# cmusphinx/pocketsphinx

Measured on NVIDIA H100. Metric: frames/sec senone-eval+Viterbi, higher is better.
Workload: dtype f32->i16/i32

## Files before the change

### pocketsphinx_b200/csrc/psb_hmm.cu

```cuda
#include "psb_hmmctx.cuh"

#include <stdlib.h>
#include <string.h>

#include <algorithm>

#include <vector>


struct psb_phoneloop_s {
    psb_hmmctx_t *c;
    int n_phones, window, beam, pbeam, pip;
    double penalty_weight;
    Stream stream;
    DevBuf<int32_t> d_ssid, d_tmatid;
    DevBuf<uint16_t> d_senid;
    DevBuf<int32_t> d_flags;
};

namespace {

__device__ __forceinline__ void load_hmm(const psb_hmm_t *p, HmmReg &h, int n)
{
#pragma unroll
    for (int i = 0; i < PSB_HMM_MAX_NSTATE; ++i) {
        h.score[i] = i < n ? p->score[i] : PSB_WORST_SCORE;
        h.hist[i] = i < n ? p->history[i] : -1;
        h.senid[i] = i < n ? p->senid[i] : PSB_BAD_SSID;
    }
    h.out_score = p->out_score;
    h.out_hist = p->out_history;
    h.best = p->bestscore;
}

__device__ __forceinline__ void store_hmm(psb_hmm_t *p, const HmmReg &h, int n, bool mpx)
{
#pragma unroll
    for (int i = 0; i < PSB_HMM_MAX_NSTATE; ++i)
        if (i < n) {
            p->score[i] = h.score[i];
            p->history[i] = h.hist[i];
            if (mpx) p->senid[i] = (uint16_t)h.senid[i];
        }
    p->out_score = h.out_score;
    p->out_history = h.out_hist;
    p->bestscore = h.best;
}

__global__ void __launch_bounds__(256)
hmm_eval_aos_kernel(psb_hmm_t *hmms, int n, HmmCtxDev c, const int16_t *__restrict__ senscr, int *best_out)
{
    __shared__ int red[8];
    const int i = blockIdx.x * blockDim.x + threadIdx.x;
    int best = PSB_WORST_SCORE;
    if (i < n) {
        psb_hmm_t *p = hmms + i;
        HmmReg h;
        load_hmm(p, h, c.n_emit);
        const bool mpx = p->mpx != 0;
        best = hmm_step(h, c, p->tmatid, mpx, senscr);
        store_hmm(p, h, c.n_emit, mpx);
    }
    best = __reduce_max_sync(0xffffffffu, best);
    if ((threadIdx.x & 31) == 0) red[threadIdx.x >> 5] = best;
    __syncthreads();
    if (threadIdx.x < 32) {
        int v = threadIdx.x < (blockDim.x >> 5) ? red[threadIdx.x] : PSB_WORST_SCORE;
        v = __reduce_max_sync(0xffffffffu, v);
        if (threadIdx.x == 0) atomicMax(best_out, v);
    }
}

struct PlParams {
    int n_phones, window, beam, pbeam, pip;
    double penalty_weight;
};

template <typename T>
__device__ __forceinline__ T block_reduce_max_pair(T v, int idx, int *sidx, T *sval, int &out_idx)
{
    const unsigned full = 0xffffffffu;
#pragma unroll
    for (int o = 16; o > 0; o >>= 1) {
        T ov = __shfl_xor_sync(full, v, o);
        int oi = __shfl_xor_sync(full, idx, o);
        if (ov > v || (ov == v && oi < idx)) { v = ov; idx = oi; }
    }
    const int warp = threadIdx.x >> 5, lane = threadIdx.x & 31, nw = blockDim.x >> 5;
// ... 294 lines not shown
{
    if (!p) return;
    cudaSetDevice(p->c->device);
    cudaStreamSynchronize(p->stream);
    delete p;
}

int psb_phoneloop_launch(psb_phoneloop_t *p, const int16_t *d_senscr, const int32_t *d_utt_off, int32_t n_utt,
                         int32_t *d_best, int32_t *d_pen, psb_hmm_t *d_final, psb_hmm_t *d_trace, cudaStream_t st)
{
    const int H = p->n_phones, N = p->c->n_emit;
    size_t smem = ((size_t)(2 * N + 4 + p->window) * H + 64) * sizeof(int);
    PSB_REQUIRE(smem <= 227 * 1024, "phone loop with %d HMMs needs %zu bytes of shared memory (max 227 KB)", H, smem);
    PSB_CUDA(cudaFuncSetAttribute(phoneloop_kernel, cudaFuncAttributeMaxDynamicSharedMemorySize, (int)smem));
    int threads = std::min(1024, roundup(H, 32));
    PlParams P;
    P.n_phones = H; P.window = p->window; P.beam = p->beam; P.pbeam = p->pbeam; P.pip = p->pip;
    P.penalty_weight = p->penalty_weight;
    phoneloop_kernel<<<n_utt, threads, smem, st>>>(d_senscr, d_utt_off, dev_ctx(p->c), P, p->d_senid, p->d_tmatid, p->d_ssid,
                                                   d_best, d_pen, d_final, d_trace, p->d_flags);
    PSB_LAUNCH_CHECK();
    return PSB_OK;
}

int psb_phoneloop_n_phones(const psb_phoneloop_t *p) { return p->n_phones; }

extern "C" int psb_phoneloop_run_device(psb_phoneloop_t *p, const int16_t *d_senscr, const int32_t *utt_off,
                                        int32_t n_utt, int32_t *d_best, int32_t *d_pen, psb_hmm_t *final_hmms,
                                        void *batch)
{
    PSB_REQUIRE(p && d_senscr && utt_off && n_utt >= 0, "psb_phoneloop_run_device: bad argument");
    if (n_utt == 0) return PSB_OK;
    int rc = ctx_check_utts("psb_phoneloop_run_device", utt_off, n_utt, d_senscr);
    if (rc) return rc;
    PSB_CUDA(cudaSetDevice(p->c->device));
    cudaStream_t st = batch ? psb_batch_stream((psb_batch_t *)batch) : p->stream;
    DevBuf<int32_t> d_off;
    DevBuf<psb_hmm_t> d_final;
    if ((rc = d_off.reserve((size_t)n_utt + 1))) return rc;
    if (final_hmms && (rc = d_final.reserve((size_t)n_utt * p->n_phones))) return rc;
    PSB_CUDA(cudaMemcpyAsync(d_off, utt_off, (size_t)(n_utt + 1) * 4, cudaMemcpyHostToDevice, st));
    rc = psb_phoneloop_launch(p, d_senscr, d_off, n_utt, d_best, d_pen, d_final, nullptr, st);
    if (!rc && final_hmms) {
        cudaError_t e = cudaMemcpyAsync(final_hmms, d_final, (size_t)n_utt * p->n_phones * sizeof(psb_hmm_t),
                                        cudaMemcpyDeviceToHost, st);
        if (e != cudaSuccess) { psb_set_error("%s", cudaGetErrorString(e)); rc = PSB_ERR_CUDA; }
    }
    cudaStreamSynchronize(st);
    return rc;
}

extern "C" int psb_phoneloop_run_host(psb_phoneloop_t *p, const int16_t *senscr, const int32_t *utt_off, int32_t n_utt,
                                      int32_t *best, int32_t *pen, psb_hmm_t *hmm_trace)
{
    PSB_REQUIRE(p && senscr && utt_off && n_utt >= 0, "psb_phoneloop_run_host: bad argument");
    if (n_utt == 0) return PSB_OK;
    int rc = ctx_check_utts("psb_phoneloop_run_host", utt_off, n_utt, senscr);
    if (rc) return rc;
    PSB_CUDA(cudaSetDevice(p->c->device));
    const size_t total = utt_off[n_utt], H = p->n_phones;
    DevBuf<int16_t> d_scr;
    DevBuf<int32_t> d_off, d_best, d_pen;
    DevBuf<psb_hmm_t> d_tr;
    if ((rc = d_scr.reserve(std::max<size_t>(1, total * p->c->n_sen))) || (rc = d_off.reserve((size_t)n_utt + 1)) ||
        (best && (rc = d_best.reserve(std::max<size_t>(1, total)))) || (pen && (rc = d_pen.reserve(std::max<size_t>(1, total * H)))) ||
        (hmm_trace && (rc = d_tr.reserve(std::max<size_t>(1, total * H)))))
        return rc;
    cudaError_t e = cudaMemcpy(d_scr, senscr, total * p->c->n_sen * 2, cudaMemcpyHostToDevice);
    if (e == cudaSuccess) e = cudaMemcpy(d_off, utt_off, (size_t)(n_utt + 1) * 4, cudaMemcpyHostToDevice);
    if (e == cudaSuccess) {
        rc = psb_phoneloop_launch(p, d_scr, d_off, n_utt, d_best, d_pen, nullptr, d_tr, p->stream);
        if (!rc) e = cudaStreamSynchronize(p->stream);
        if (!rc && e == cudaSuccess && best) e = cudaMemcpy(best, d_best, total * 4, cudaMemcpyDeviceToHost);
        if (!rc && e == cudaSuccess && pen) e = cudaMemcpy(pen, d_pen, total * H * 4, cudaMemcpyDeviceToHost);
        if (!rc && e == cudaSuccess && hmm_trace)
            e = cudaMemcpy(hmm_trace, d_tr, total * H * sizeof(psb_hmm_t), cudaMemcpyDeviceToHost);
    }
    if (e != cudaSuccess) { psb_set_error("psb_phoneloop_run_host: %s", cudaGetErrorString(e)); rc = PSB_ERR_CUDA; }
    return rc;
}

constexpr int HS_V = 4;
constexpr int HS_TS = 512;
constexpr int SWEEP_FR = 2;

struct psb_hmmset_s {
    psb_hmmctx_t *c;
    int64_t n_max, n, pitch;
    int32_t n_seg_max, n_seg;
    int64_t max_seg_len;
    bool any_mpx;
    Stream own_stream;
    cudaStream_t stream;
    DevBuf<int32_t> d_i32;
    DevBuf<uint16_t> d_u16;
    DevBuf<uint8_t> d_mpx;
    DevBuf<int64_t> d_seg_off;
    DevBuf<int64_t> d_seg_base;
    DevBuf<psb_hmm_t> d_aos;
    DevBuf<int32_t> d_snap_i32;
    Event ev[2];
};

namespace {

struct HmmSetDev {
    int32_t *i32;
    uint16_t *u16;
    uint8_t *mpx;
    const int64_t *seg_off, *seg_base;
    int64_t pitch;
    int n_seg;
};

static HmmSetDev dev_set(const psb_hmmset_t *s)
{
    HmmSetDev d;
    d.i32 = s->d_i32; d.u16 = s->d_u16; d.mpx = s->d_mpx; d.seg_off = s->d_seg_off; d.seg_base = s->d_seg_base;
    d.pitch = s->pitch; d.n_seg = s->n_seg;
    return d;
}

template <bool TO_SOA>
__global__ void __launch_bounds__(256)
hmmset_convert_kernel(psb_hmm_t *aos, HmmSetDev s, int64_t n, int ns)
{
    const int64_t a = (int64_t)blockIdx.x * blockDim.x + threadIdx.x;
    if (a >= n) return;
    int lo = 0, hi = s.n_seg;
    while (hi - lo > 1) {
        const int mid = (lo + hi) >> 1;
        if (s.seg_off[mid] <= a) lo = mid; else hi = mid;
    }
    const int64_t i = s.seg_base[lo] + (a - s.seg_off[lo]);
    psb_hmm_t *p = aos + a;
    const int64_t b32 = (i / HS_TS) * (int64_t)(2 * ns + 4) * HS_TS + (i % HS_TS);
    const int64_t b16 = (i / HS_TS) * (int64_t)(ns + 2) * HS_TS + (i % HS_TS);
    int32_t *score = s.i32 + b32, *hist = score + ns * HS_TS, *tail = score + 2 * ns * HS_TS;
    uint16_t *senid = s.u16 + b16, *ids = senid + ns * HS_TS;
    if (TO_SOA) {
        for (int k = 0; k < ns; ++k) {
            score[k * HS_TS] = p->score[k];
            hist[k * HS_TS] = p->history[k];
            senid[k * HS_TS] = p->senid[k];
        }
        tail[0] = p->out_score; tail[HS_TS] = p->out_history; tail[2 * HS_TS] = p->bestscore; tail[3 * HS_TS] = p->frame;
        ids[0] = p->ssid; ids[HS_TS] = (uint16_t)p->tmatid;
        s.mpx[i] = p->mpx;
    }
    else {
        for (int k = 0; k < PSB_HMM_MAX_NSTATE; ++k) {
            p->score[k] = k < ns ? score[k * HS_TS] : 0;
            p->history[k] = k < ns ? hist[k * HS_TS] : 0;
            p->senid[k] = k < ns ? senid[k * HS_TS] : 0;
        }
        p->out_score = tail[0]; p->out_history = tail[HS_TS]; p->bestscore = tail[2 * HS_TS]; p->frame = tail[3 * HS_TS];
        p->ssid = ids[0]; p->tmatid = (int16_t)ids[HS_TS];
        p->mpx = s.mpx[i]; p->n_emit_state = (uint8_t)ns;
        p->ctx = nullptr;
    }
}

__global__ void fill_i32_kernel(int32_t *p, int64_t n, int32_t v)
{
    const int64_t i = (int64_t)blockIdx.x * blockDim.x + threadIdx.x;
    if (i < n) p[i] = v;
}
// ... 96 lines not shown
            reinterpret_cast<int16_t *>(dst + head + body)[threadIdx.x - 32] = row[((head + body) >> 1) + threadIdx.x - 32];
        srow_al = reinterpret_cast<const int16_t *>(dst);
        __syncthreads();
        if (body) mbar_wait(&row_bar, 0u);
    }
    int best = PSB_WORST_SCORE;
    if (live) {
        bool any_mpx = false;
#pragma unroll
        for (int q = 0; q < HS_V; ++q) {
            HmmReg h;
#pragma unroll
            for (int k = 0; k < PSB_HMM_MAX_NSTATE; ++k) {
                const bool in = k < NL && k < ns;
                h.score[k] = in ? comp(sc[k < NL ? k : 0], q) : PSB_WORST_SCORE;
                h.hist[k] = in ? comp(hi[k < NL ? k : 0], q) : -1;
                const unsigned w = (q < 2) ? sid[k < NL ? k : 0].x : sid[k < NL ? k : 0].y;
                h.senid[k] = in ? (int)((q & 1) ? (w >> 16) : (w & 0xffffu)) : PSB_BAD_SSID;
            }
            h.out_score = comp(osc, q);
            h.out_hist = comp(ohi, q);
            h.best = PSB_WORST_SCORE;
            const unsigned tw = (q < 2) ? tm.x : tm.y;
            const int tmatid = (int16_t)((q & 1) ? (tw >> 16) : (tw & 0xffffu));
            const bool mpx = (q == 0 ? mp.x : q == 1 ? mp.y : q == 2 ? mp.z : mp.w) != 0;
            const int b = hmm_step(h, c, tmatid, mpx, srow_al);
            if (j0 + q < n) best = max(best, b);
#pragma unroll
            for (int k = 0; k < NL; ++k)
                if (k < ns) {
                    setc(sc[k], q, h.score[k]);
                    setc(hi[k], q, h.hist[k]);
                    if (mpx) {
                        unsigned &w = (q < 2) ? sid[k].x : sid[k].y;
                        w = (q & 1) ? ((w & 0xffffu) | ((unsigned)h.senid[k] << 16)) : ((w & 0xffff0000u) | ((unsigned)h.senid[k] & 0xffffu));
                        any_mpx = true;
                    }
                }
            setc(osc, q, h.out_score);
            setc(ohi, q, h.out_hist);
            setc(bst, q, h.best);
        }
#pragma unroll
        for (int k = 0; k < NL; ++k)
            if (k < ns) {
                __stcs(reinterpret_cast<int4 *>(score + k * HS_TS), sc[k]);
                __stcs(reinterpret_cast<int4 *>(hist + k * HS_TS), hi[k]);
                if (any_mpx) __stcs(reinterpret_cast<uint2 *>(senid + k * HS_TS), sid[k]);
            }
        __stcs(reinterpret_cast<int4 *>(tail), osc);
        __stcs(reinterpret_cast<int4 *>(tail + HS_TS), ohi);
        __stcs(reinterpret_cast<int4 *>(tail + 2 * HS_TS), bst);
    }
    best = __reduce_max_sync(0xffffffffu, best);
    if ((threadIdx.x & 31) == 0) red[threadIdx.x >> 5] = best;
    __syncthreads();
    if (threadIdx.x < 32) {
        int v = threadIdx.x < (HS_THREADS >> 5) ? red[threadIdx.x] : PSB_WORST_SCORE;
        v = __reduce_max_sync(0xffffffffu, v);
        if (threadIdx.x == 0) atomicMax(best_out + seg, v);
    }
}

__device__ __forceinline__ unsigned cluster_ctarank() { unsigned r; asm volatile("mov.u32 %0, %%cluster_ctarank;" : "=r"(r)); return r; }
__device__ __forceinline__ unsigned cluster_nctarank() { unsigned r; asm volatile("mov.u32 %0, %%cluster_nctarank;" : "=r"(r)); return r; }
__device__ __forceinline__ unsigned mapa_shared(const void *p, unsigned rank)
{
    unsigned r;
    asm volatile("mapa.shared::cluster.u32 %0, %1, %2;" : "=r"(r) : "r"((unsigned)__cvta_generic_to_shared(p)), "r"(rank));
    return r;
}
__device__ __forceinline__ void st_cluster_u32(unsigned addr, unsigned v) { asm volatile("st.shared::cluster.u32 [%0], %1;" :: "r"(addr), "r"(v) : "memory"); }
__device__ __forceinline__ unsigned ld_cluster_u32(unsigned addr) { unsigned v; asm volatile("ld.shared::cluster.u32 %0, [%1];" : "=r"(v) : "r"(addr) : "memory"); return v; }
__device__ __forceinline__ void st_async_v2(unsigned remote_addr, unsigned a, unsigned b, unsigned remote_bar)
{
    asm volatile("st.async.weak.shared::cluster.mbarrier::complete_tx::bytes.v2.b32 [%0], {%1, %2}, [%3];"
                 :: "r"(remote_addr), "r"(a), "r"(b), "r"(remote_bar) : "memory");
}
__device__ __forceinline__ void cluster_sync_all()
{
    asm volatile("barrier.cluster.arrive.release.aligned;\n\tbarrier.cluster.wait.acquire.aligned;" ::: "memory");
}

template <int NS, int V, int THREADS, bool BEAM>
__global__ void __launch_bounds__(THREADS, BEAM ? 1 : 2)
hmmset_sweep_kernel(HmmSetDev s, HmmCtxDev c, const int16_t *__restrict__ senscr, long long rows_total,
                    const int64_t *__restrict__ row0, const int32_t *__restrict__ n_rows, int n_frames,
                    int32_t *__restrict__ best_out, int n_tmat, int buf_bytes, int frame0, int beam, int maxhmmpf,
                    int32_t *__restrict__ n_active_out)
{
    static_assert(!BEAM || THREADS == 256, "the histogram walk maps one bin to one thread");
    constexpr int FR = BEAM ? 1 : SWEEP_FR;
    constexpr int NBUF = BEAM ? 6 : 2 * FR;
    extern __shared__ __align__(128) unsigned char sw_smem[];
    __shared__ __align__(8) uint64_t full[NBUF];
    __shared__ int red[2 * FR][THREADS / 32];
    __shared__ int redc[BEAM ? 2 : 1][THREADS / 32];
    __shared__ __align__(8) int2 cl_slot[BEAM ? 2 : 1][16];
    __shared__ __align__(8) uint64_t xbar[2];
    __shared__ unsigned hist[BEAM ? 2 : 1][BEAM ? 256 : 1];
    __shared__ unsigned scan_w[8];
    __shared__ int found;
    const int seg = blockIdx.y, tid = threadIdx.x;
    const int64_t n = s.seg_off[seg + 1] - s.seg_off[seg];
    const int64_t j_base = (int64_t)blockIdx.x * THREADS * V;
    const bool cta_empty = j_base >= n;
    if (!BEAM && cta_empty) return;
    int T = n_frames;
    if (n_rows) T = min(T, n_rows[seg]);
    if (T <= 0) return;
    const unsigned my_rank = BEAM ? cluster_ctarank() : 0u, n_rank = BEAM ? cluster_nctarank() : 1u;
    if (BEAM) {
        hist[0][tid] = 0u;
        hist[1][tid] = 0u;
        if (tid == 0) {
            mbar_init(&xbar[0], 1);
            mbar_init(&xbar[1], 1);
            asm volatile("fence.mbarrier_init.release.cluster;" ::: "memory");
        }
    }
    uint8_t *tps = sw_smem + NBUF * (size_t)buf_bytes;
    for (int q = tid; q < n_tmat * NS * (NS + 1); q += THREADS) tps[q] = c.tp[q];

    int sc[V][NS], hi[V][NS], sid[V][NS], osc[V], ohi[V], tmo[V];
    HmmTp3 tk[V];
    bool live[V], act[V], touched[V];
    const int64_t rem64 = n - j_base - tid;
    const int rem = rem64 < 0 ? -1 : rem64 > V * THREADS ? V * THREADS : (int)rem64;
    auto state_i32 = [&](int v) {
        const int64_t j = j_base + (int64_t)v * THREADS + tid;
        const int64_t i = s.seg_base[seg] + (j < n ? j : 0);
        return s.i32 + (i / HS_TS) * (int64_t)(2 * NS + 4) * HS_TS + (i % HS_TS);
    };
#pragma unroll
    for (int v = 0; v < V; ++v) {
        const int64_t j = j_base + (int64_t)v * THREADS + tid;
        live[v] = j < n;
        const int64_t i = s.seg_base[seg] + (live[v] ? j : 0);
        const int64_t b16 = (i / HS_TS) * (int64_t)(NS + 2) * HS_TS + (i % HS_TS);
        const int32_t *p32 = state_i32(v);
        const uint16_t *p16 = s.u16 + b16;
#pragma unroll
        for (int k = 0; k < NS; ++k) {
            sc[v][k] = live[v] ? p32[k * HS_TS] : PSB_WORST_SCORE;
            hi[v][k] = live[v] ? p32[(NS + k) * HS_TS] : -1;
            sid[v][k] = live[v] ? 2 * (int)p16[k * HS_TS] : 0;
        }
        osc[v] = live[v] ? p32[2 * NS * HS_TS] : PSB_WORST_SCORE;
        ohi[v] = live[v] ? p32[(2 * NS + 1) * HS_TS] : -1;
        tmo[v] = live[v] ? (int)(int16_t)p16[(NS + 1) * HS_TS] * NS * (NS + 1) : 0;
        act[v] = BEAM ? (live[v] && p32[(2 * NS + 3) * HS_TS] == frame0) : live[v];
        touched[v] = act[v];
    }
    __syncthreads();
    if (NS == 3) {
#pragma unroll
        for (int v = 0; v < V; ++v) tk[v] = hmm_tp3_decode(tps + tmo[v]);
    }
    const int64_t r0 = row0 ? row0[seg] : seg;
    const int64_t rstep = row0 ? 1 : gridDim.y;
    const size_t row_bytes = (size_t)c.n_sen * 2;
    auto row_addr = [&](int t) { return reinterpret_cast<uintptr_t>(senscr + (size_t)(r0 + (int64_t)t * rstep) * c.n_sen); };
    const int64_t lim = rows_total - 1 - r0;
    const int t_tma = lim <= 0 ? 0 : (int)min((int64_t)T, (lim + rstep - 1) / rstep);
    auto tma_ok = [&](int t) { return t < t_tma; };
    const unsigned a_lo0 = (unsigned)row_addr(0), a_step = (unsigned)((size_t)rstep * row_bytes);
    if (BEAM) cluster_sync_all();
    auto issue = [&](int t) {
        const uintptr_t a = row_addr(t), a16 = a & ~(uintptr_t)15;
        const unsigned bytes = (unsigned)(((a - a16) + row_bytes + 15) & ~(size_t)15);
        mbar_expect_tx(&full[t % NBUF], bytes);
        tma_bulk_g2s(sw_smem + (size_t)(t % NBUF) * buf_bytes, reinterpret_cast<const void *>(a16), bytes, &full[t % NBUF]);
    };
    if (tid == 0) {
        for (int q = 0; q < NBUF; ++q) mbar_init(&full[q], 1);
        asm volatile("fence.mbarrier_init.release.cluster;" ::: "memory");
    }
    __syncthreads();
    if (tid == 0 && !cta_empty)
        for (int q = 0; q < NBUF && q < T; ++q)
            if (tma_ok(q)) issue(q);
    int best_final[V];
#pragma unroll
    for (int v = 0; v < V; ++v) best_final[v] = PSB_WORST_SCORE;

    for (int t = 0; t < T; ++t) {
        const int b = t & 1, rb = t % NBUF;
        unsigned char *buf = sw_smem + (size_t)rb * buf_bytes;
        const int16_t *srow;
        if (BEAM && cta_empty)
            srow = reinterpret_cast<const int16_t *>(buf);
        else if (tma_ok(t)) {
            mbar_wait(&full[rb], (unsigned)(t / NBUF) & 1u);
            srow = reinterpret_cast<const int16_t *>(buf + ((a_lo0 + (unsigned)t * a_step) & 15u));
        }
        else {
            const int16_t *g = reinterpret_cast<const int16_t *>(row_addr(t));
            int16_t *d = reinterpret_cast<int16_t *>(buf);
            for (int q = tid; q < c.n_sen; q += THREADS) d[q] = g[q];
            __syncthreads();
            srow = d;
        }
        const unsigned char *srowb = reinterpret_cast<const unsigned char *>(srow);
        auto score_at = [&](int off) { return (int)*reinterpret_cast<const int16_t *>(srowb + off); };
        int best = PSB_WORST_SCORE, cnt = 0;
#pragma unroll
        for (int v = 0; v < V; ++v) {
            if (BEAM && !act[v]) continue;
            ++cnt;
            int bb;
            if (NS == 3) {
                int (&s3)[3] = *reinterpret_cast<int (*)[3]>(sc[v]);
                int (&h3)[3] = *reinterpret_cast<int (*)[3]>(hi[v]);
                bb = hmm_step_3st_dec(s3, h3, osc[v], ohi[v], tk[v], score_at(sid[v][0]), score_at(sid[v][1]),
                                      score_at(sid[v][NS > 2 ? 2 : 0]));
            }
            else {
                HmmReg h;
                int obs[PSB_HMM_MAX_NSTATE];
#pragma unroll
                for (int k = 0; k < PSB_HMM_MAX_NSTATE; ++k) {
                    h.score[k] = k < NS ? sc[v][k < NS ? k : 0] : PSB_WORST_SCORE;
                    h.hist[k] = k < NS ? hi[v][k < NS ? k : 0] : -1;
                    h.senid[k] = 0;
                    obs[k] = k < NS ? -score_at(sid[v][k < NS ? k : 0]) : 0;
                }
                h.out_score = osc[v]; h.out_hist = ohi[v]; h.best = PSB_WORST_SCORE;
                bb = hmm_step_5st(h, tps + tmo[v], obs);
#pragma unroll
                for (int k = 0; k < NS; ++k) { sc[v][k] = h.score[k]; hi[v][k] = h.hist[k]; }
                osc[v] = h.out_score; ohi[v] = h.out_hist;
            }
            if (v * THREADS < rem) best = max(best, bb);
            best_final[v] = bb;
        }
        best = __reduce_max_sync(0xffffffffu, best);
        if (BEAM) cnt = __reduce_add_sync(0xffffffffu, cnt);
        const int slot = t % (2 * FR);
        if ((tid & 31) == 0) {
            red[slot][tid >> 5] = best;
            if (BEAM) redc[b][tid >> 5] = cnt;
        }
        if (FR > 1 && t % FR != FR - 1 && t + 1 < T) continue;
        const int tf = t - t % FR;
        __syncthreads();
        if (tid == 0 && !cta_empty)
#pragma unroll 1
            for (int u = tf + NBUF; u <= t + NBUF; ++u)
                if (u < T && tma_ok(u)) issue(u);
        if (tid < 32) {
            if (!BEAM) {
#pragma unroll 1
                for (int u = tf; u <= t; ++u) {
                    int v = tid < THREADS / 32 ? red[u % (2 * FR)][tid] : PSB_WORST_SCORE;
                    v = __reduce_max_sync(0xffffffffu, v);
                    if (tid == 0) atomicMax(best_out + (size_t)u * gridDim.y + seg, v);
                }
            }
            else {
                int v = tid < THREADS / 32 ? red[slot][tid] : PSB_WORST_SCORE;
                v = __reduce_max_sync(0xffffffffu, v);
                int cc = tid < THREADS / 32 ? redc[b][tid] : 0;
                cc = __reduce_add_sync(0xffffffffu, cc);
                if (tid == 0) mbar_expect_tx(&xbar[b], n_rank * 8u);
                if ((unsigned)tid < n_rank)
                    st_async_v2(mapa_shared(&cl_slot[b][my_rank], (unsigned)tid), (unsigned)v, (unsigned)cc,
                                mapa_shared(&xbar[b], (unsigned)tid));
            }
        }
        if (BEAM) {
            mbar_wait(&xbar[b], (unsigned)(t >> 1) & 1u);
            int seg_best = PSB_WORST_SCORE, seg_cnt = 0;
            for (unsigned r = 0; r < n_rank; ++r) {
                const int2 m = cl_slot[b][r];
                seg_best = max(seg_best, m.x);
                seg_cnt += m.y;
            }
            if (my_rank == 0 && tid == 0) {
                best_out[(size_t)t * gridDim.y + seg] = seg_best;
                if (n_active_out) n_active_out[(size_t)t * gridDim.y + seg] = seg_cnt;
            }
            hist[b ^ 1][tid] = 0u;
            int dyn = beam;
            if (maxhmmpf >= 0 && seg_cnt > maxhmmpf) {
                const int bw = -beam / 256;
#pragma unroll
                for (int v = 0; v < V; ++v)
                    if (act[v]) {
                        int bin = (seg_best - best_final[v]) / bw;
                        bin = bin > 255 ? 255 : bin;
                        atomicAdd(&hist[b][bin], 1u);
                    }
                if (tid == 0) found = 256;
                cluster_sync_all();
                unsigned tot = 0;
                for (unsigned r = 0; r < n_rank; ++r) tot += ld_cluster_u32(mapa_shared(&hist[b][tid], r));
                unsigned incl = tot;
#pragma unroll
                for (int o = 1; o < 32; o <<= 1) {
                    const unsigned y = __shfl_up_sync(0xffffffffu, incl, o);
                    if ((tid & 31) >= o) incl += y;
                }
                if ((tid & 31) == 31) scan_w[tid >> 5] = incl;
                __syncthreads();
                for (int w = 0; w < (tid >> 5); ++w) incl += scan_w[w];
                if (incl > (unsigned)maxhmmpf) atomicMin(&found, tid);
                __syncthreads();
                dyn = -(found * bw);
            }
            const int thresh = seg_best + dyn;
#pragma unroll
            for (int v = 0; v < V; ++v)
                if (act[v] && !(best_final[v] > thresh)) {
#pragma unroll
                    for (int k = 0; k < NS; ++k) { sc[v][k] = PSB_WORST_SCORE; hi[v][k] = -1; }
                    osc[v] = PSB_WORST_SCORE; ohi[v] = -1; best_final[v] = PSB_WORST_SCORE;
                    act[v] = false;
                }
// ... 124 lines not shown
    PSB_CUDA(cudaMemsetAsync(s->d_mpx, 0, (size_t)s->pitch, s->stream));
    if (n) {
        PSB_CUDA(cudaMemcpyAsync(s->d_aos, hmms, (size_t)n * sizeof(psb_hmm_t), cudaMemcpyHostToDevice, s->stream));
        hmmset_convert_kernel<true><<<(unsigned)((n + 255) / 256), 256, 0, s->stream>>>(s->d_aos, dev_set(s), n, ns);
        PSB_LAUNCH_CHECK();
    }
    PSB_CUDA(cudaStreamSynchronize(s->stream));
    return PSB_OK;
}

extern "C" int psb_hmmset_download(psb_hmmset_t *s, psb_hmm_t *hmms)
{
    PSB_REQUIRE(s && (s->n == 0 || hmms), "psb_hmmset_download: bad argument");
    if (s->n == 0) return PSB_OK;
    PSB_CUDA(cudaSetDevice(s->c->device));
    int rc = hmmset_staging(s);
    if (rc) return rc;
    hmmset_convert_kernel<false><<<(unsigned)((s->n + 255) / 256), 256, 0, s->stream>>>(s->d_aos, dev_set(s), s->n, s->c->n_emit);
    PSB_LAUNCH_CHECK();
    std::vector<psb_hmm_t> tmp((size_t)s->n);
    PSB_CUDA(cudaMemcpyAsync(tmp.data(), s->d_aos, (size_t)s->n * sizeof(psb_hmm_t), cudaMemcpyDeviceToHost, s->stream));
    PSB_CUDA(cudaStreamSynchronize(s->stream));
    for (int64_t i = 0; i < s->n; ++i) {
        void *ctx = hmms[i].ctx;
        hmms[i] = tmp[(size_t)i];
        hmms[i].ctx = ctx;
    }
    return PSB_OK;
}

extern "C" int psb_hmmset_eval_frames_device(psb_hmmset_t *s, const int16_t *d_senscr, const int64_t *d_row0,
                                             const int32_t *d_n_rows, int32_t n_frames, int32_t *d_best, float *ms)
{
    PSB_REQUIRE(s && d_senscr && d_best && n_frames >= 0, "psb_hmmset_eval_frames_device: bad argument");
    if (ms) *ms = 0.f;
    if (n_frames == 0 || s->n_seg == 0) return PSB_OK;
    PSB_CUDA(cudaSetDevice(s->c->device));
    const int64_t nb = (int64_t)n_frames * s->n_seg;
    fill_i32_kernel<<<(unsigned)((nb + 255) / 256), 256, 0, s->stream>>>(d_best, nb, PSB_WORST_SCORE);
    PSB_LAUNCH_CHECK();
    if (s->n == 0) {
        PSB_CUDA(cudaStreamSynchronize(s->stream));
        return PSB_OK;
    }
    static const int threads = [] {
        const char *v = getenv("PSB_HMMSET_THREADS");
        return v && atoi(v) == 256 ? 256 : 128;
    }();
    const int tile = threads * HS_V;
    const dim3 grid((unsigned)((s->max_seg_len + tile - 1) / tile), (unsigned)s->n_seg);
    const HmmSetDev sd = dev_set(s);
    const HmmCtxDev cd = dev_ctx(s->c);
    const size_t smem = (((size_t)cd.n_sen * 2 + 15) & ~(size_t)15) + 16;
    PSB_REQUIRE(smem <= 200 * 1024, "psb_hmmset: %d senones do not fit the shared-memory score row", cd.n_sen);
    auto launch = [&](auto kern, int t, int32_t *best) {
        kern<<<grid, threads, smem, s->stream>>>(sd, cd, d_senscr, d_row0, d_n_rows, t, best);
    };
#define PSB_HS_ATTR(NS, NT) PSB_CUDA(cudaFuncSetAttribute(hmmset_eval_kernel<NS, NT>, cudaFuncAttributeMaxDynamicSharedMemorySize, (int)smem))
    if (smem > 48 * 1024) {
        PSB_HS_ATTR(3, 256); PSB_HS_ATTR(5, 256); PSB_HS_ATTR(0, 256); PSB_HS_ATTR(3, 128); PSB_HS_ATTR(5, 128); PSB_HS_ATTR(0, 128);
    }
#undef PSB_HS_ATTR
    PSB_CUDA(cudaEventRecord(s->ev[0], s->stream));
    for (int t = 0; t < n_frames; ++t) {
        int32_t *best = d_best + (size_t)t * s->n_seg;
        if (threads == 256) {
            if (cd.n_emit == 3) launch(hmmset_eval_kernel<3, 256>, t, best);
            else if (cd.n_emit == 5) launch(hmmset_eval_kernel<5, 256>, t, best);
            else launch(hmmset_eval_kernel<0, 256>, t, best);
        }
        else {
            if (cd.n_emit == 3) launch(hmmset_eval_kernel<3, 128>, t, best);
            else if (cd.n_emit == 5) launch(hmmset_eval_kernel<5, 128>, t, best);
            else launch(hmmset_eval_kernel<0, 128>, t, best);
        }
        PSB_LAUNCH_CHECK();
    }
    PSB_CUDA(cudaEventRecord(s->ev[1], s->stream));
    PSB_CUDA(cudaStreamSynchronize(s->stream));
    if (ms) PSB_CUDA(cudaEventElapsedTime(ms, s->ev[0], s->ev[1]));
    return PSB_OK;
}

extern "C" int psb_hmmset_sweep_device(psb_hmmset_t *s, const int16_t *d_senscr, int64_t rows_total, const int64_t *d_row0,
                                       const int32_t *d_n_rows, int32_t n_frames, int32_t *d_best, float *ms)
{
    PSB_REQUIRE(s && d_senscr && d_best && n_frames >= 0 && rows_total > 0, "psb_hmmset_sweep_device: bad argument");
    const HmmCtxDev cd = dev_ctx(s->c);
    if (s->any_mpx || (cd.n_emit != 3 && cd.n_emit != 5) || (cd.n_sen & 1))
        return psb_hmmset_eval_frames_device(s, d_senscr, d_row0, d_n_rows, n_frames, d_best, ms);
    if (ms) *ms = 0.f;
    if (n_frames == 0 || s->n_seg == 0) return PSB_OK;
    PSB_CUDA(cudaSetDevice(s->c->device));
    const int64_t nb = (int64_t)n_frames * s->n_seg;
    fill_i32_kernel<<<(unsigned)((nb + 255) / 256), 256, 0, s->stream>>>(d_best, nb, PSB_WORST_SCORE);
    PSB_LAUNCH_CHECK();
    if (s->n == 0) {
        if (ms) PSB_CUDA(cudaStreamSynchronize(s->stream));
        return PSB_OK;
    }
    const int buf_bytes = (int)(((size_t)cd.n_sen * 2 + 32 + 127) & ~(size_t)127);
    const int tp_bytes = s->c->n_tmat * cd.n_emit * (cd.n_emit + 1);
    const size_t smem = 2 * SWEEP_FR * (size_t)buf_bytes + tp_bytes;
    PSB_REQUIRE(smem <= 200 * 1024, "psb_hmmset_sweep: %d senones / %d transition matrices do not fit shared memory", cd.n_sen, s->c->n_tmat);
    const HmmSetDev sd = dev_set(s);
    PSB_CUDA(cudaEventRecord(s->ev[0], s->stream));
#define PSB_SWEEP(NS, V, THREADS)                                                                                               \
    do {                                                                                                                       \
        auto kern = hmmset_sweep_kernel<NS, V, THREADS, false>;                                                                \
        PSB_CUDA(cudaFuncSetAttribute(kern, cudaFuncAttributeMaxDynamicSharedMemorySize, (int)smem));                          \
        const dim3 grid((unsigned)((s->max_seg_len + THREADS * V - 1) / (THREADS * V)), (unsigned)s->n_seg);                   \
        kern<<<grid, THREADS, smem, s->stream>>>(sd, cd, d_senscr, (long long)rows_total, d_row0, d_n_rows, n_frames, d_best,  \
                                                s->c->n_tmat, buf_bytes, 0, 0, -1, nullptr);                                   \
    } while (0)
    if (cd.n_emit == 3) PSB_SWEEP(3, 4, 256);
    else PSB_SWEEP(5, 4, 256);
#undef PSB_SWEEP
    PSB_LAUNCH_CHECK();
    PSB_CUDA(cudaEventRecord(s->ev[1], s->stream));
    if (ms) {
        PSB_CUDA(cudaStreamSynchronize(s->stream));
        PSB_CUDA(cudaEventElapsedTime(ms, s->ev[0], s->ev[1]));
    }
    return PSB_OK;
}

extern "C" int psb_hmmset_sweep_beam_device(psb_hmmset_t *s, const int16_t *d_senscr, int64_t rows_total, const int64_t *d_row0,
                                            const int32_t *d_n_rows, int32_t n_frames, int32_t frame0, int32_t beam,
                                            int32_t maxhmmpf, int32_t *d_best, int32_t *d_n_active, float *ms)
{
    PSB_REQUIRE(s && d_senscr && d_best && n_frames >= 0 && rows_total > 0, "psb_hmmset_sweep_beam_device: bad argument");
    PSB_REQUIRE(beam < 0 && beam > -0x20000000, "psb_hmmset_sweep_beam_device: the beam is a negative log score (got %d)", beam);
    PSB_REQUIRE(maxhmmpf < 0 || beam <= -256, "psb_hmmset_sweep_beam_device: -maxhmmpf needs a beam of at least 256 score units (bin width -beam/256)");
    const HmmCtxDev cd = dev_ctx(s->c);
    PSB_REQUIRE(!s->any_mpx && (cd.n_emit == 3 || cd.n_emit == 5) && !(cd.n_sen & 1),
                "psb_hmmset_sweep_beam_device: plain 3- or 5-state instances and an even senone count (the fused kernel's shapes)");
    constexpr int THREADS = 256, V = 4;
    const int64_t per_seg = (s->max_seg_len + THREADS * V - 1) / (THREADS * V);
    PSB_REQUIRE(per_seg <= 16, "psb_hmmset_sweep_beam_device: a segment of %lld instances needs %lld CTAs, a cluster holds 16",
                (long long)s->max_seg_len, (long long)per_seg);
    if (ms) *ms = 0.f;
    if (n_frames == 0 || s->n_seg == 0) return PSB_OK;
    PSB_CUDA(cudaSetDevice(s->c->device));
    const int64_t nb = (int64_t)n_frames * s->n_seg;
    fill_i32_kernel<<<(unsigned)((nb + 255) / 256), 256, 0, s->stream>>>(d_best, nb, PSB_WORST_SCORE);
    PSB_LAUNCH_CHECK();
    if (d_n_active) PSB_CUDA(cudaMemsetAsync(d_n_active, 0, (size_t)nb * 4, s->stream));
    if (s->n == 0) {
        if (ms) PSB_CUDA(cudaStreamSynchronize(s->stream));
        return PSB_OK;
    }
    const int buf_bytes = (int)(((size_t)cd.n_sen * 2 + 32 + 127) & ~(size_t)127);
    const int tp_bytes = s->c->n_tmat * cd.n_emit * (cd.n_emit + 1);
    const size_t smem = 6 * (size_t)buf_bytes + tp_bytes;
    PSB_REQUIRE(smem <= 200 * 1024, "psb_hmmset_sweep_beam: %d senones / %d transition matrices do not fit shared memory", cd.n_sen, s->c->n_tmat);
    const HmmSetDev sd = dev_set(s);
    const long long rows_ll = rows_total;
    const int n_tmat = s->c->n_tmat;
    cudaLaunchConfig_t cfg = {};
    cfg.gridDim = dim3((unsigned)std::max<int64_t>(per_seg, 1), (unsigned)s->n_seg);
    cfg.blockDim = dim3(THREADS);
    cfg.dynamicSmemBytes = smem;
    cfg.stream = s->stream;
    cudaLaunchAttribute at[1];
    at[0].id = cudaLaunchAttributeClusterDimension;
    at[0].val.clusterDim.x = cfg.gridDim.x; at[0].val.clusterDim.y = 1; at[0].val.clusterDim.z = 1;
    cfg.attrs = at; cfg.numAttrs = 1;
    PSB_CUDA(cudaEventRecord(s->ev[0], s->stream));
#define PSB_SWEEPB(NS)                                                                                                         \
    do {                                                                                                                       \
        auto kern = hmmset_sweep_kernel<NS, V, THREADS, true>;                                                                 \
        PSB_CUDA(cudaFuncSetAttribute(kern, cudaFuncAttributeMaxDynamicSharedMemorySize, (int)smem));                          \
        if (cfg.gridDim.x > 8) PSB_CUDA(cudaFuncSetAttribute(kern, cudaFuncAttributeNonPortableClusterSizeAllowed, 1));       \
        int n_clusters = 0;                                                                                                    \
        PSB_CUDA(cudaOccupancyMaxActiveClusters(&n_clusters, kern, &cfg));                                                     \
        PSB_REQUIRE(n_clusters > 0, "psb_hmmset_sweep_beam: a cluster of %u CTAs with %zu bytes of shared memory each does not fit the device", \
                    cfg.gridDim.x, smem);                                                                                      \
        PSB_CUDA(cudaLaunchKernelEx(&cfg, kern, sd, cd, d_senscr, rows_ll, d_row0, d_n_rows, (int)n_frames, d_best, n_tmat,   \
                                    buf_bytes, (int)frame0, (int)beam, (int)maxhmmpf, d_n_active));                            \
        PSB_LAUNCH_CHECK();                                                                                                    \
    } while (0)
    if (cd.n_emit == 3) PSB_SWEEPB(3);
    else PSB_SWEEPB(5);
#undef PSB_SWEEPB
    PSB_CUDA(cudaEventRecord(s->ev[1], s->stream));
    if (ms) {
        PSB_CUDA(cudaStreamSynchronize(s->stream));
        PSB_CUDA(cudaEventElapsedTime(ms, s->ev[0], s->ev[1]));
    }
    return PSB_OK;
}

extern "C" int psb_hmmset_eval_host(psb_hmmset_t *s, const int16_t *senscr, int32_t *best)
{
    PSB_REQUIRE(s && senscr && best, "psb_hmmset_eval_host: bad argument");
    PSB_CUDA(cudaSetDevice(s->c->device));
    DevBuf<int16_t> d_scr;
    DevBuf<int32_t> d_best;
    const size_t nb = (size_t)s->n_seg * s->c->n_sen * 2;
    int rc = d_scr.reserve(nb / 2);
    if (!rc) rc = d_best.reserve((size_t)s->n_seg);
    if (rc) return rc;
    cudaError_t e = cudaMemcpy(d_scr, senscr, nb, cudaMemcpyHostToDevice);
    if (e == cudaSuccess) {
        rc = psb_hmmset_eval_frames_device(s, d_scr, nullptr, nullptr, 1, d_best, nullptr);
        if (!rc) e = cudaMemcpy(best, d_best, (size_t)s->n_seg * 4, cudaMemcpyDeviceToHost);
    }
    if (e != cudaSuccess) {
// ... 751 lines not shown
```

### pocketsphinx_b200/csrc/psb_hmm.cuh

```cuda
#pragma once
#include "psb_internal.cuh"

struct HmmCtxDev {
    int n_emit;
    int n_sen;
    const uint8_t *tp;
    const uint16_t *sseq;
};

struct HmmReg {
    int score[PSB_HMM_MAX_NSTATE];
    int hist[PSB_HMM_MAX_NSTATE];
    int out_score, out_hist;
    int senid[PSB_HMM_MAX_NSTATE];
    int best;
};

__device__ __forceinline__ int hmm_pick3(int t0, int t1, int t2, int &out)
{
    if (t0 > t1) {
        if (t2 > t0) { out = t2; return 2; }
        out = t0; return 0;
    }
    if (t2 > t1) { out = t2; return 2; }
    out = t1; return 1;
}

#define PSB_FLOOR(s) do { if ((s) < PSB_WORST_SCORE) (s) = PSB_WORST_SCORE; } while (0)
#define PSB_RAISE(b, s) do { if ((s) > (b)) (b) = (s); } while (0)

__device__ __forceinline__ int hmm_step_3st(HmmReg &h, const uint8_t *tp, const int (&obs)[PSB_HMM_MAX_NSTATE])
{
#define TP(i, j) (-(int)tp[(i) * 4 + (j)])
    int s0, s1, s2, s3, t0, t1, t2, best = PSB_WORST_SCORE;
    s2 = h.score[2] + obs[2];
    s1 = h.score[1] + obs[1];
    s0 = h.score[0] + obs[0];
    t2 = INT_MIN;
    if (s1 > PSB_WORST_SCORE) {
        t1 = s2 + TP(2, 3);
        if (TP(1, 3) > PSB_TMAT_WORST) t2 = s1 + TP(1, 3);
        if (t1 > t2) { s3 = t1; h.out_hist = h.hist[2]; }
        else { s3 = t2; h.out_hist = h.hist[1]; }
        PSB_FLOOR(s3);
        h.out_score = s3;
        best = s3;
    }
    t0 = s2 + TP(2, 2);
    t1 = s1 + TP(1, 2);
    if (TP(0, 2) > PSB_TMAT_WORST) t2 = s0 + TP(0, 2);
    {
        int w = hmm_pick3(t0, t1, t2, s2);
        if (w == 2) h.hist[2] = h.hist[0];
        else if (w == 1) h.hist[2] = h.hist[1];
    }
    PSB_FLOOR(s2); PSB_RAISE(best, s2);
    h.score[2] = s2;
    t0 = s1 + TP(1, 1);
    t1 = s0 + TP(0, 1);
    if (t0 > t1) s1 = t0;
    else { s1 = t1; h.hist[1] = h.hist[0]; }
    PSB_FLOOR(s1); PSB_RAISE(best, s1);
    h.score[1] = s1;
    s0 = s0 + TP(0, 0);
    PSB_FLOOR(s0); PSB_RAISE(best, s0);
    h.score[0] = s0;
    h.best = best;
    return best;
#undef TP
}

struct HmmTp3 {
    int p00, p01, p11, p12, p22, p23, p02, p13;
    int m02, m13;
};

__device__ __forceinline__ HmmTp3 hmm_tp3_decode(const uint8_t *tp)
{
    HmmTp3 k;
    k.p00 = -(int)tp[0]; k.p01 = -(int)tp[1]; k.p02 = -(int)tp[2];
    k.p11 = -(int)tp[5]; k.p12 = -(int)tp[6]; k.p13 = -(int)tp[7];
    k.p22 = -(int)tp[10]; k.p23 = -(int)tp[11];
    asm("mov.b32 %0, %1;" : "=r"(k.m02) : "r"(k.p02 > PSB_TMAT_WORST ? -1 : 0));
    asm("mov.b32 %0, %1;" : "=r"(k.m13) : "r"(k.p13 > PSB_TMAT_WORST ? -1 : 0));
    return k;
}

__device__ __forceinline__ int hmm_msel(int m, int a, int b) { return (a & m) | (b & ~m); }

__device__ __forceinline__ int hmm_step_3st_dec(int (&sc)[3], int (&hi)[3], int &osc, int &ohi, const HmmTp3 &k,
                                                int x0, int x1, int x2)
{
    const int s2 = sc[2] - x2, s1 = sc[1] - x1, s0 = sc[0] - x0;
    const bool a = s1 > PSB_WORST_SCORE;
    const int e1 = s2 + k.p23;
    const int e2 = hmm_msel(k.m13, s1 + k.p13, INT_MIN);
    const int s3 = max(max(e1, e2), PSB_WORST_SCORE);
    const int oh = e1 > e2 ? hi[2] : hi[1];
    osc = a ? s3 : osc;
    ohi = a ? oh : ohi;
    const int u2 = hmm_msel(k.m02, s0 + k.p02, a ? e2 : INT_MIN);
    const int u0 = s2 + k.p22, u1 = s1 + k.p12;
    const int m01 = max(u0, u1);
    const int n2 = max(max(m01, u2), PSB_WORST_SCORE);
    const int h2 = u2 > m01 ? hi[0] : (u0 > u1 ? hi[2] : hi[1]);
    const int v0 = s1 + k.p11, v1 = s0 + k.p01;
    const int n1 = max(max(v0, v1), PSB_WORST_SCORE);
    const int h1 = v0 > v1 ? hi[1] : hi[0];
    const int n0 = max(s0 + k.p00, PSB_WORST_SCORE);
    sc[0] = n0; sc[1] = n1; sc[2] = n2;
    hi[1] = h1; hi[2] = h2;
    return max(max(a ? s3 : PSB_WORST_SCORE, n2), max(n1, n0));
}

__device__ __forceinline__ int hmm_step_5st(HmmReg &h, const uint8_t *tp, const int (&obs)[PSB_HMM_MAX_NSTATE])
{
#define TP(i, j) (-(int)tp[(i) * 6 + (j)])
    int s0, s1, s2, s3, s4, s5, t0, t1, t2, best = PSB_WORST_SCORE;
    s4 = h.score[4] + obs[4];
    s3 = h.score[3] + obs[3];
    if (s3 > PSB_WORST_SCORE) {
        t1 = s4 + TP(4, 5);
        t2 = s3 + TP(3, 5);
        if (t1 > t2) { s5 = t1; h.out_hist = h.hist[4]; }
        else { s5 = t2; h.out_hist = h.hist[3]; }
        PSB_FLOOR(s5);
        h.out_score = s5;
        best = s5;
    }
    s2 = h.score[2] + obs[2];
    if (s2 > PSB_WORST_SCORE) {
        int w = hmm_pick3(s4 + TP(4, 4), s3 + TP(3, 4), s2 + TP(2, 4), s4);
        if (w == 2) h.hist[4] = h.hist[2];
        else if (w == 1) h.hist[4] = h.hist[3];
        PSB_FLOOR(s4); PSB_RAISE(best, s4);
        h.score[4] = s4;
    }
    s1 = h.score[1] + obs[1];
    if (s1 > PSB_WORST_SCORE) {
        int w = hmm_pick3(s3 + TP(3, 3), s2 + TP(2, 3), s1 + TP(1, 3), s3);
        if (w == 2) h.hist[3] = h.hist[1];
        else if (w == 1) h.hist[3] = h.hist[2];
        PSB_FLOOR(s3); PSB_RAISE(best, s3);
        h.score[3] = s3;
    }
    s0 = h.score[0] + obs[0];
    {
        int w = hmm_pick3(s2 + TP(2, 2), s1 + TP(1, 2), s0 + TP(0, 2), s2);
        if (w == 2) h.hist[2] = h.hist[0];
        else if (w == 1) h.hist[2] = h.hist[1];
        PSB_FLOOR(s2); PSB_RAISE(best, s2);
        h.score[2] = s2;
    }
    t0 = s1 + TP(1, 1);
    t1 = s0 + TP(0, 1);
    if (t0 > t1) s1 = t0;
    else { s1 = t1; h.hist[1] = h.hist[0]; }
    PSB_FLOOR(s1); PSB_RAISE(best, s1);
    h.score[1] = s1;
    s0 = s0 + TP(0, 0);
    PSB_FLOOR(s0); PSB_RAISE(best, s0);
    h.score[0] = s0;
    h.best = best;
    return best;
#undef TP
}

__device__ __forceinline__ int mpx_obs(const HmmCtxDev &c, const int16_t *senscr, const HmmReg &h, int st)
{
    return -(int)senscr[c.sseq[(size_t)h.senid[st] * c.n_emit + st]];
}

__device__ __forceinline__ int hmm_step_3st_mpx(HmmReg &h, const HmmCtxDev &c, const uint8_t *tp, const int16_t *senscr)
{
#define TP(i, j) (-(int)tp[(i) * 4 + (j)])
    int s0, s1, s2, s3, t0, t1, t2, best, w;
    t2 = INT_MIN;
// ... 209 lines not shown
```

Baseline: 12.35 million.

## Specialize 3-state sweep with warp-uniform live fast path and larger blocks

The non-beam sweep kernel now runs 512 threads per block and stages four frames per sync instead of two, with launch bounds derived from the thread count. For 3-state HMMs it drops the per-lane liveness test on the best-score max by giving padding lanes transition values that can never win. Each frame it also checks warp-wide whether every state-1 score is live and, if so, runs a specialised step that skips the conditional selects. It adds a compile-time candidate dispatcher for tuning, plus more shared memory per block and an extra warp vote per frame.

```diff
diff --git a/pocketsphinx_b200/csrc/psb_hmm.cu b/pocketsphinx_b200/csrc/psb_hmm.cu
--- a/pocketsphinx_b200/csrc/psb_hmm.cu
+++ b/pocketsphinx_b200/csrc/psb_hmm.cu
@@ -4,6 +4,7 @@
 #include <string.h>
 
 #include <algorithm>
+#include <type_traits>
 
 #include <vector>
 
@@ -464,7 +465,7 @@
 
 constexpr int HS_V = 4;
 constexpr int HS_TS = 512;
-constexpr int SWEEP_FR = 2;
+constexpr int SWEEP_FR = 4;
 
 struct psb_hmmset_s {
     psb_hmmctx_t *c;
@@ -727,15 +728,15 @@
     asm volatile("barrier.cluster.arrive.release.aligned;\n\tbarrier.cluster.wait.acquire.aligned;" ::: "memory");
 }
 
-template <int NS, int V, int THREADS, bool BEAM>
-__global__ void __launch_bounds__(THREADS, BEAM ? 1 : 2)
+template <int NS, int V, int THREADS, bool BEAM, int FRP = SWEEP_FR, bool LIVE_TEST = (NS != 3), bool FAST = (NS == 3 && !BEAM)>
+__global__ void __launch_bounds__(THREADS, BEAM || THREADS >= 512 || V > 4 ? 1 : 512 / THREADS)
 hmmset_sweep_kernel(HmmSetDev s, HmmCtxDev c, const int16_t *__restrict__ senscr, long long rows_total,
                     const int64_t *__restrict__ row0, const int32_t *__restrict__ n_rows, int n_frames,
                     int32_t *__restrict__ best_out, int n_tmat, int buf_bytes, int frame0, int beam, int maxhmmpf,
                     int32_t *__restrict__ n_active_out)
 {
     static_assert(!BEAM || THREADS == 256, "the histogram walk maps one bin to one thread");
-    constexpr int FR = BEAM ? 1 : SWEEP_FR;
+    constexpr int FR = BEAM ? 1 : FRP;
     constexpr int NBUF = BEAM ? 6 : 2 * FR;
     extern __shared__ __align__(128) unsigned char sw_smem[];
     __shared__ __align__(8) uint64_t full[NBUF];
@@ -800,7 +801,7 @@
     __syncthreads();
     if (NS == 3) {
 #pragma unroll
-        for (int v = 0; v < V; ++v) tk[v] = hmm_tp3_decode(tps + tmo[v]);
+        for (int v = 0; v < V; ++v) tk[v] = live[v] ? hmm_tp3_decode(tps + tmo[v]) : hmm_tp3_padding();
     }
     const int64_t r0 = row0 ? row0[seg] : seg;
     const int64_t rstep = row0 ? 1 : gridDim.y;
@@ -849,6 +850,14 @@
         const unsigned char *srowb = reinterpret_cast<const unsigned char *>(srow);
         auto score_at = [&](int off) { return (int)*reinterpret_cast<const int16_t *>(srowb + off); };
         int best = PSB_WORST_SCORE, cnt = 0;
+        bool s1_live = false;
+        if (NS == 3 && FAST) {
+            bool all = true;
+#pragma unroll
+            for (int v = 0; v < V; ++v) all &= sc[v][1] - score_at(sid[v][1]) > PSB_WORST_SCORE;
+            s1_live = __all_sync(0xffffffffu, all);
+        }
+        auto frame_steps = [&](auto s1_known) {
 #pragma unroll
         for (int v = 0; v < V; ++v) {
             if (BEAM && !act[v]) continue;
@@ -857,7 +866,7 @@
             if (NS == 3) {
                 int (&s3)[3] = *reinterpret_cast<int (*)[3]>(sc[v]);
                 int (&h3)[3] = *reinterpret_cast<int (*)[3]>(hi[v]);
-                bb = hmm_step_3st_dec(s3, h3, osc[v], ohi[v], tk[v], score_at(sid[v][0]), score_at(sid[v][1]),
+                bb = hmm_step_3st_dec<decltype(s1_known)::value>(s3, h3, osc[v], ohi[v], tk[v], score_at(sid[v][0]), score_at(sid[v][1]),
                                       score_at(sid[v][NS > 2 ? 2 : 0]));
             }
             else {
@@ -876,9 +885,12 @@
                 for (int k = 0; k < NS; ++k) { sc[v][k] = h.score[k]; hi[v][k] = h.hist[k]; }
                 osc[v] = h.out_score; ohi[v] = h.out_hist;
             }
-            if (v * THREADS < rem) best = max(best, bb);
+            if (!LIVE_TEST || v * THREADS < rem) best = max(best, bb);
             best_final[v] = bb;
         }
+        };
+        if (NS == 3 && FAST && s1_live) frame_steps(std::true_type());
+        else frame_steps(std::false_type());
         best = __reduce_max_sync(0xffffffffu, best);
         if (BEAM) cnt = __reduce_add_sync(0xffffffffu, cnt);
         const int slot = t % (2 * FR);
@@ -1169,8 +1181,28 @@
     return PSB_OK;
 }
 
-extern "C" int psb_hmmset_sweep_device(psb_hmmset_t *s, const int16_t *d_senscr, int64_t rows_total, const int64_t *d_row0,
-                                       const int32_t *d_n_rows, int32_t n_frames, int32_t *d_best, float *ms)
+template <int NS, int V, int THREADS, int FR, bool LIVE_TEST = (NS != 3), bool FAST = (NS == 3)>
+static int sweep_launch(psb_hmmset_t *s, const int16_t *d_senscr, int64_t rows_total, const int64_t *d_row0,
+                        const int32_t *d_n_rows, int32_t n_frames, int32_t *d_best)
+{
+    const HmmCtxDev cd = dev_ctx(s->c);
+    const int buf_bytes = (int)(((size_t)cd.n_sen * 2 + 32 + 127) & ~(size_t)127);
+    const int tp_bytes = s->c->n_tmat * NS * (NS + 1);
+    const size_t smem = 2 * FR * (size_t)buf_bytes + tp_bytes;
+    PSB_REQUIRE(smem <= 200 * 1024, "psb_hmmset_sweep: %d senones / %d transition matrices do not fit shared memory", cd.n_sen, s->c->n_tmat);
+    auto kern = hmmset_sweep_kernel<NS, V, THREADS, false, FR, LIVE_TEST, FAST>;
+    PSB_CUDA(cudaFuncSetAttribute(kern, cudaFuncAttributeMaxDynamicSharedMemorySize, (int)smem));
+    const dim3 grid((unsigned)((s->max_seg_len + THREADS * V - 1) / (THREADS * V)), (unsigned)s->n_seg);
+    PSB_CUDA(cudaEventRecord(s->ev[0], s->stream));
+    kern<<<grid, THREADS, smem, s->stream>>>(dev_set(s), cd, d_senscr, (long long)rows_total, d_row0, d_n_rows, n_frames, d_best,
+                                            s->c->n_tmat, buf_bytes, 0, 0, -1, nullptr);
+    PSB_LAUNCH_CHECK();
+    PSB_CUDA(cudaEventRecord(s->ev[1], s->stream));
+    return PSB_OK;
+}
+
+static int sweep_device(psb_hmmset_t *s, const int16_t *d_senscr, int64_t rows_total, const int64_t *d_row0,
+                        const int32_t *d_n_rows, int32_t n_frames, int32_t *d_best, int candidate, float *ms)
 {
     PSB_REQUIRE(s && d_senscr && d_best && n_frames >= 0 && rows_total > 0, "psb_hmmset_sweep_device: bad argument");
     const HmmCtxDev cd = dev_ctx(s->c);
@@ -1186,31 +1218,42 @@
         if (ms) PSB_CUDA(cudaStreamSynchronize(s->stream));
         return PSB_OK;
     }
-    const int buf_bytes = (int)(((size_t)cd.n_sen * 2 + 32 + 127) & ~(size_t)127);
-    const int tp_bytes = s->c->n_tmat * cd.n_emit * (cd.n_emit + 1);
-    const size_t smem = 2 * SWEEP_FR * (size_t)buf_bytes + tp_bytes;
-    PSB_REQUIRE(smem <= 200 * 1024, "psb_hmmset_sweep: %d senones / %d transition matrices do not fit shared memory", cd.n_sen, s->c->n_tmat);
-    const HmmSetDev sd = dev_set(s);
-    PSB_CUDA(cudaEventRecord(s->ev[0], s->stream));
-#define PSB_SWEEP(NS, V, THREADS)                                                                                               \
-    do {                                                                                                                       \
-        auto kern = hmmset_sweep_kernel<NS, V, THREADS, false>;                                                                \
-        PSB_CUDA(cudaFuncSetAttribute(kern, cudaFuncAttributeMaxDynamicSharedMemorySize, (int)smem));                          \
-        const dim3 grid((unsigned)((s->max_seg_len + THREADS * V - 1) / (THREADS * V)), (unsigned)s->n_seg);                   \
-        kern<<<grid, THREADS, smem, s->stream>>>(sd, cd, d_senscr, (long long)rows_total, d_row0, d_n_rows, n_frames, d_best,  \
-                                                s->c->n_tmat, buf_bytes, 0, 0, -1, nullptr);                                   \
-    } while (0)
-    if (cd.n_emit == 3) PSB_SWEEP(3, 4, 256);
-    else PSB_SWEEP(5, 4, 256);
-#undef PSB_SWEEP
-    PSB_LAUNCH_CHECK();
-    PSB_CUDA(cudaEventRecord(s->ev[1], s->stream));
+    int rc;
+    if (cd.n_emit == 5) rc = sweep_launch<5, 4, 512, SWEEP_FR>(s, d_senscr, rows_total, d_row0, d_n_rows, n_frames, d_best);
+#ifdef PSB_SWEEP_CANDIDATES
+    else if (candidate == 1) rc = sweep_launch<3, 4, 256, 2>(s, d_senscr, rows_total, d_row0, d_n_rows, n_frames, d_best);
+    else if (candidate == 2) rc = sweep_launch<3, 4, 512, 1>(s, d_senscr, rows_total, d_row0, d_n_rows, n_frames, d_best);
+    else if (candidate == 3) rc = sweep_launch<3, 4, 512, 4, false, false>(s, d_senscr, rows_total, d_row0, d_n_rows, n_frames, d_best);
+    else if (candidate == 4) rc = sweep_launch<3, 4, 512, 8>(s, d_senscr, rows_total, d_row0, d_n_rows, n_frames, d_best);
+    else if (candidate == 5) rc = sweep_launch<3, 4, 256, 2, true, false>(s, d_senscr, rows_total, d_row0, d_n_rows, n_frames, d_best);
+    else if (candidate == 6) rc = sweep_launch<3, 4, 512, 2, true, false>(s, d_senscr, rows_total, d_row0, d_n_rows, n_frames, d_best);
+    else if (candidate == 7) rc = sweep_launch<3, 4, 512, 2>(s, d_senscr, rows_total, d_row0, d_n_rows, n_frames, d_best);
+    else if (candidate == 8) rc = sweep_launch<3, 4, 256, 4>(s, d_senscr, rows_total, d_row0, d_n_rows, n_frames, d_best);
+#endif
+    else rc = sweep_launch<3, 4, 512, SWEEP_FR>(s, d_senscr, rows_total, d_row0, d_n_rows, n_frames, d_best);
+    (void)candidate;
+    if (rc) return rc;
     if (ms) {
         PSB_CUDA(cudaStreamSynchronize(s->stream));
         PSB_CUDA(cudaEventElapsedTime(ms, s->ev[0], s->ev[1]));
     }
     return PSB_OK;
 }
+
+extern "C" int psb_hmmset_sweep_device(psb_hmmset_t *s, const int16_t *d_senscr, int64_t rows_total, const int64_t *d_row0,
+                                       const int32_t *d_n_rows, int32_t n_frames, int32_t *d_best, float *ms)
+{
+    return sweep_device(s, d_senscr, rows_total, d_row0, d_n_rows, n_frames, d_best, 0, ms);
+}
+
+#ifdef PSB_SWEEP_CANDIDATES
+extern "C" int psb_hmmset_sweep_candidate_device(psb_hmmset_t *s, const int16_t *d_senscr, int64_t rows_total, const int64_t *d_row0,
+                                                 const int32_t *d_n_rows, int32_t n_frames, int32_t *d_best, int32_t candidate,
+                                                 float *ms)
+{
+    return sweep_device(s, d_senscr, rows_total, d_row0, d_n_rows, n_frames, d_best, candidate, ms);
+}
+#endif
 
 extern "C" int psb_hmmset_sweep_beam_device(psb_hmmset_t *s, const int16_t *d_senscr, int64_t rows_total, const int64_t *d_row0,
                                             const int32_t *d_n_rows, int32_t n_frames, int32_t frame0, int32_t beam,
diff --git a/pocketsphinx_b200/csrc/psb_hmm.cuh b/pocketsphinx_b200/csrc/psb_hmm.cuh
--- a/pocketsphinx_b200/csrc/psb_hmm.cuh
+++ b/pocketsphinx_b200/csrc/psb_hmm.cuh
@@ -86,13 +86,23 @@
     return k;
 }
 
+__device__ __forceinline__ HmmTp3 hmm_tp3_padding()
+{
+    constexpr int PAD = -0x100000;
+    HmmTp3 k;
+    k.p00 = k.p01 = k.p02 = k.p11 = k.p12 = k.p13 = k.p22 = k.p23 = PAD;
+    k.m02 = k.m13 = -1;
+    return k;
+}
+
 __device__ __forceinline__ int hmm_msel(int m, int a, int b) { return (a & m) | (b & ~m); }
 
+template <bool S1_LIVE = false>
 __device__ __forceinline__ int hmm_step_3st_dec(int (&sc)[3], int (&hi)[3], int &osc, int &ohi, const HmmTp3 &k,
                                                 int x0, int x1, int x2)
 {
     const int s2 = sc[2] - x2, s1 = sc[1] - x1, s0 = sc[0] - x0;
-    const bool a = s1 > PSB_WORST_SCORE;
+    const bool a = S1_LIVE || s1 > PSB_WORST_SCORE;
     const int e1 = s2 + k.p23;
     const int e2 = hmm_msel(k.m13, s1 + k.p13, INT_MIN);
     const int s3 = max(max(e1, e2), PSB_WORST_SCORE);
```

New measurement: 12.82 million (median of 6 runs). 1.04x the previous value.
